# hmorimitsu/ptlflow

Measured on AMD Instinct MI355X. Metric: frame-pairs/sec, RAFT 32-iter 436x1024, higher is better.
Workload: dtype f32; 1 GPU; raft random-init (seeded), 436x1024 frame pairs, 32 iterations, fp32, batch 8/GPU, eval forward incl. encoders, mask head + convex upsample on every iteration as the reference; global_batch=8, parallelism=dp1 (independent replicas, no collectives)

## Files before the change

### include/pfk.h

```cpp
#ifndef PFK_H
#define PFK_H

#include <stdint.h>

#ifdef __cplusplus
extern "C" {
#endif

typedef void* pfk_stream_t;

enum pfk_status {
  PFK_OK = 0,
  PFK_ERR_BAD_ARG = -1,
  PFK_ERR_ALIGNMENT = -2,
  PFK_ERR_UNSUPPORTED = -3,
  PFK_ERR_LAUNCH = -4,
  PFK_ERR_DISABLED = -5
};

#define PFK_MAX_LEVELS 8
#define PFK_ABI_VERSION 7

int pfk_abi_version(void);
const char* pfk_status_string(int status);
// ... 106 lines not shown
  long long workspace_bytes;
  int cout_active;
  int cout_split;
} pfk_conv_desc;

long long pfk_conv_workspace_bytes(void);
long long pfk_conv_workspace_fault_offset(void);
int pfk_conv_ktot(const pfk_conv_desc* d);
int pfk_conv2d_f32(const pfk_conv_desc* d, pfk_stream_t stream);

#define PFK_CONV_GROUP_MAX 4
int pfk_conv2d_group_f32(const pfk_conv_desc* descs, int n, pfk_stream_t stream);

long long pfk_conv_wino_weight_floats(int cin, int cout);
int pfk_conv2d_wino_f32(const pfk_conv_desc* d, pfk_stream_t stream);

int pfk_conv2d_wino_res_f32(const pfk_conv_desc* d, pfk_stream_t stream);

int pfk_conv2d_wino_norm_f32(const pfk_conv_desc* d, const float* in_mean, const float* in_rstd, int in_relu, pfk_stream_t stream);

long long pfk_conv_wino_stats_workspace_bytes(int B, int H, int W, int cout);
int pfk_conv2d_wino_stats_f32(const pfk_conv_desc* d, const float* in_mean, const float* in_rstd, int in_relu, float eps,
                              float* out_mean, float* out_rstd, void* workspace, long long workspace_bytes, pfk_stream_t stream);

long long pfk_conv_wino1d_weight_floats(int ktot, int cout);
int pfk_conv1d_wino_f32(const pfk_conv_desc* d, pfk_stream_t stream);

int pfk_conv_ktot_bf16(const pfk_conv_desc* d);
int pfk_conv2d_bf16s(const pfk_conv_desc* d, const void* weight_planes, int nsplit, pfk_stream_t stream);

typedef struct {
  const void* ptr;
  int ld;
  int channels;
} pfk_conv_src_b16;

typedef struct {
  pfk_conv_src_b16 src[3];
  int num_src;
  int B, H, W;
  int kh, kw;
  const void* weight;
  const float* bias;
  int cout;
  int epilogue;
  int relu;
// ... 190 lines not shown
```

### ptlflow_amd/csrc/pfk_torch.cpp

```cpp
#include <torch/library.h>

#include <type_traits>
#include <vector>

#include "pfk_torch_views.h"

namespace {

void corr_volume_impl(const char* op, Elem e, const Tensor& f1, const Tensor& f2, double scale, const Tensor& out) {
  OpScope scope(f1);
  const Ptr a = dense(op, f1, "f1", e), b = dense(op, f2, "f2", e), o = dense(op, out, "out", e);
  TORCH_CHECK(f1.dim() == 3 && f2.dim() == 3 && out.dim() == 3, op, ": [B,N,D] inputs, [B,N1,N2] out");
  const int B = f1.size(0), N1 = f1.size(1), D = f1.size(2), N2 = f2.size(1);
  TORCH_CHECK(f2.size(0) == B && f2.size(2) == D && out.size(0) == B && out.size(1) == N1 && out.size(2) == N2, op, ": shape mismatch");
  if (e == B16) check_ok(pfk_corr_volume_bf16(a.raw(), D, b.raw(), D, o.raw(), B, N1, N2, D, (float)scale, cur_stream()), op);
  else check_ok(pfk_corr_volume_f32(a.f32(), D, b.f32(), D, o.f32(), B, N1, N2, D, (float)scale, cur_stream()), op);
}
void corr_volume(const Tensor& f1, const Tensor& f2, double scale, Tensor out) { corr_volume_impl("corr_volume", F32, f1, f2, scale, out); }
void corr_volume_bf16(const Tensor& f1, const Tensor& f2, double scale, Tensor out) { corr_volume_impl("corr_volume_bf16", B16, f1, f2, scale, out); }

void corr_pool2x2(const Tensor& in, Tensor out) {
  OpScope scope(in);
  const Ptr i = dense("corr_pool2x2", in, "inp", Any);
  TORCH_CHECK(in.dim() == 3, "corr_pool2x2: inp must be [M,H,W] contiguous");
// ... 286 lines not shown
  }
  check_ok(pfk_conv2d_b16(&d, cur_stream()), "conv2d_b16");
}

void conv2d_b16(at::TensorList srcs, int64_t B, int64_t H, int64_t W, int64_t kh, int64_t kw, const Tensor& weight,
                const c10::optional<Tensor>& bias, int64_t cout, int64_t epilogue, bool relu, double scale,
                const c10::optional<Tensor>& out, const c10::optional<Tensor>& h, const c10::optional<Tensor>& h_b16,
                const c10::optional<Tensor>& aux_z, const c10::optional<Tensor>& aux_rh, const c10::optional<Tensor>& residual,
                int64_t stride, bool relu_after_residual) {
  conv2d_b16_run(srcs, B, H, W, kh, kw, weight, bias, cout, epilogue, relu, scale, out, h, h_b16, aux_z, aux_rh, residual, stride,
                 relu_after_residual, false);
}

void conv2d_gelu_b16(at::TensorList srcs, int64_t B, int64_t H, int64_t W, int64_t kh, int64_t kw, const Tensor& weight,
                     const c10::optional<Tensor>& bias, int64_t cout, double scale, const Tensor& out,
                     const c10::optional<Tensor>& residual) {
  TORCH_CHECK(weight.dim() == 2, "conv2d_gelu_b16: bf16 packed weight [cout, ktot] (no batched form)");
  conv2d_b16_run(srcs, B, H, W, kh, kw, weight, bias, cout, PFK_EPI_LINEAR_GELU, false, scale, out, c10::nullopt, c10::nullopt,
                 c10::nullopt, c10::nullopt, residual, 1, false, true);
}

void debug_set_b16(int64_t cfg) { check_ok(pfk_debug_set_b16((int)cfg), "debug_set_b16"); }
void debug_set_stem_valu(int64_t on) { check_ok(pfk_debug_set_stem_valu((int)on), "debug_set_stem_valu"); }
void debug_set_cin2_valu(int64_t on) { check_ok(pfk_debug_set_cin2_valu((int)on), "debug_set_cin2_valu"); }

void conv_cin2(const Tensor& in, const Tensor& weight, const c10::optional<Tensor>& bias, Tensor out,
               int64_t B, int64_t H, int64_t W, int64_t k, bool relu) {
  OpScope scope(in);
  const Rows i = rows("conv_cin2", in, "inp", F32).expect(B * H * W, AtLeast{2});
  const Rows o = rows("conv_cin2", out, "out", Any).expect(B * H * W, AtLeast{0});
  const int cout = o.cols;
  const float* wp = dense("conv_cin2", weight, "weight [k*k,2,cout]", F32, k * k * 2 * cout).f32();
  const float* bp = dense("conv_cin2", bias, "bias", F32, AtLeast{cout}).f32();
  if (o.b16) check_ok(pfk_conv_cin2_b16(i.f32(), i.ld, wp, bp, o.raw(), o.ld, 0, B, H, W, k, cout, relu, cur_stream()), "conv_cin2 (bf16 out)");
  else check_ok(pfk_conv_cin2_f32(i.f32(), i.ld, wp, bp, o.f32(), o.ld, 0, B, H, W, k, cout, relu, cur_stream()), "conv_cin2");
}

void flow_delta(const Tensor& in, const Tensor& weight, const c10::optional<Tensor>& bias, const Tensor& coords0,
                Tensor coords1, const c10::optional<Tensor>& delta_out, const c10::optional<Tensor>& flow_out,
                const c10::optional<Tensor>& flow_out_b16) {
  OpScope scope(in);
  const float* c0 = dense("flow_delta", coords0, "coords0", F32).f32();
  TORCH_CHECK(coords0.dim() == 4 && coords0.size(1) == 2, "flow_delta: coords0 must be [B,2,h,w] contiguous");
  const int B = coords0.size(0), H = coords0.size(2), W = coords0.size(3);
  const int64_t M = (int64_t)B * H * W;
  float* c1 = dense("flow_delta", coords1, "coords1", F32, 2 * M).f32();
// ... 710 lines not shown
  m.def("corr_lookup_blocked(Tensor[] levels, int[] lvl_h, int[] lvl_w, Tensor coords, int radius, Tensor(a!) out) -> ()");
  m.def("blocked_map_elems(int H, int W) -> int", &blocked_map_elems);
  m.def("conv2d(Tensor[] srcs, int B, int H, int W, int kh, int kw, Tensor weight, Tensor? bias, int cout, "
        "int epilogue, bool relu, float scale, Tensor(a!)? out, Tensor(b!)? h, Tensor(c!)? aux_z, Tensor(d!)? aux_rh, "
        "Tensor(e!)? workspace=None, Tensor? residual=None, int stride=1, bool relu_after_residual=False, int cout_active=0, int cout_split=0) -> ()");
  m.def("conv2d_wino(Tensor src, int B, int H, int W, Tensor weight, Tensor? bias, int cout, bool relu, float scale, Tensor(a!) out, "
        "int cout_active=0) -> ()");
  m.def("conv2d_wino_norm(Tensor src, int B, int H, int W, Tensor weight, Tensor? bias, int cout, bool relu, float scale, Tensor(a!) out, "
        "Tensor in_mean, Tensor in_rstd, bool in_relu) -> ()");
  m.def("conv_wino_stats_workspace_bytes(int B, int H, int W, int cout) -> int", &conv_wino_stats_workspace_bytes);
  m.def("conv2d_wino_stats(Tensor src, int B, int H, int W, Tensor weight, Tensor? bias, int cout, Tensor(a!) out, Tensor? in_mean, "
        "Tensor? in_rstd, bool in_relu, float eps, Tensor(b!) out_mean, Tensor(c!) out_rstd, Tensor(d!) workspace) -> ()");
  m.def("conv2d_wino1d(Tensor[] srcs, int B, int H, int W, int kh, int kw, Tensor weight, Tensor? bias, int cout, int epilogue, "
        "bool relu, float scale, Tensor(a!)? out=None, Tensor(b!)? h=None, Tensor(c!)? aux_z=None, Tensor(d!)? aux_rh=None, "
        "Tensor? residual=None) -> ()");
  m.def("conv2d_wino_res(Tensor src, int B, int H, int W, Tensor weight, Tensor? bias, int cout, bool relu, float scale, Tensor(a!) out, "
        "Tensor residual, bool relu_after_residual) -> ()");
  m.def("conv2d_group(Tensor[] srcs, int B, int H, int W, int[] k, Tensor[] weights, Tensor[] biases, int[] relu, float[] scale, Tensor(a!)[] outs, Tensor[] residuals) -> ()");
  m.def("conv2d_b16(Tensor[] srcs, int B, int H, int W, int kh, int kw, Tensor weight, Tensor? bias, int cout, int epilogue, bool relu, "
        "float scale, Tensor(a!)? out, Tensor(b!)? h=None, Tensor(c!)? h_b16=None, Tensor(d!)? aux_z=None, Tensor(e!)? aux_rh=None, "
        "Tensor? residual=None, int stride=1, bool relu_after_residual=False) -> ()");
  m.def("debug_set_b16(int cfg) -> ()", &debug_set_b16);
  m.def("debug_set_stem_valu(int on) -> ()", &debug_set_stem_valu);
  m.def("debug_set_cin2_valu(int on) -> ()", &debug_set_cin2_valu);
  m.def("conv_workspace_bytes() -> int", &conv_workspace_bytes);
  m.def("conv_workspace_fault_offset() -> int", &conv_workspace_fault_offset);
  m.def("conv_cin2(Tensor inp, Tensor weight, Tensor? bias, Tensor(a!) out, int B, int H, int W, int k, bool relu) -> ()");
  m.def("flow_delta(Tensor inp, Tensor weight, Tensor? bias, Tensor coords0, Tensor(a!) coords1, Tensor(b!)? delta_out, "
        "Tensor(c!)? flow_out, Tensor(d!)? flow_out_b16=None) -> ()");
  m.def("flow_from_coords(Tensor coords0, Tensor coords1, Tensor(a!) flow_out) -> ()");
  m.def("convex_upsample(Tensor flow, Tensor mask, Tensor(a!) out) -> ()");
  m.def("convex_upsample_pm(Tensor flow_pm, Tensor mask, Tensor(a!) out) -> ()");
  m.def("convex_upsample_info_pm(Tensor flow_pm, Tensor info_pm, Tensor mask, Tensor(a!) flow_out, Tensor(b!) info_out) -> ()");
  m.def("dwconv_layernorm(Tensor inp, Tensor dw_weight, Tensor? dw_bias, Tensor ln_weight, Tensor ln_bias, float eps, Tensor(a!) out, "
        "int B, int H, int W, int k) -> ()");
  m.def("dwconv_layernorm_train(Tensor inp, Tensor dw_weight, Tensor? dw_bias, Tensor ln_weight, Tensor ln_bias, float eps, "
        "Tensor(a!) out, Tensor(b!) xhat, Tensor(c!) rstd, int B, int H, int W, int k) -> ()");
  m.def("layernorm_bwd(Tensor xhat, Tensor rstd, Tensor ln_weight, Tensor dy, Tensor(a!) du, Tensor(b!) dgamma, Tensor(c!) dbeta) -> ()");
  m.def("dwconv_bwd(Tensor inp, Tensor du, Tensor dw_weight, Tensor(a!) dx, Tensor(b!) dweight, Tensor(c!)? dbias, int B, int H, int W, "
        "int k) -> ()");
  m.def("gelu(Tensor x, Tensor(a!) y) -> ()");
  m.def("gelu_bwd(Tensor x, Tensor dy, Tensor(a!) dx) -> ()");
  m.def("dwconv_layernorm_b16(Tensor inp, Tensor dw_weight, Tensor? dw_bias, Tensor ln_weight, Tensor ln_bias, float eps, "
        "Tensor(a!) out, int B, int H, int W, int k) -> ()");
  m.def("conv2d_gelu_b16(Tensor[] srcs, int B, int H, int W, int kh, int kw, Tensor weight, Tensor? bias, int cout, float scale, "
        "Tensor(a!) out, Tensor? residual=None) -> ()");
// ... 78 lines not shown
```

### ptlflow_amd/csrc/pfk_wino.hip

```cpp
#include "pfk_gemm.h"

using namespace pfkg;

namespace {

constexpr int WT = 32;
constexpr int WN = 64;
constexpr int WK = 8;
constexpr int UIMG = 16 * WN * WK;

typedef float f32x2 __attribute__((ext_vector_type(2)));
typedef __attribute__((address_space(3))) float lfloat;
typedef __attribute__((address_space(3))) f32x2 lf32x2;
typedef __attribute__((address_space(3))) f32x4 lf32x4;

struct WinoArgs {
  const float* src; int ld;
  unsigned src_bytes;
  int H, W;
  int tw, tpi;
  int ntiles;
  int nks;
  const float* weight; unsigned w_bytes;
  const float* bias;
  int cout;
  int ncb;
  int relu; float scale;
  float* out; int out_ld, out_coff;
  unsigned out_bytes;
  const float* res; int res_ld;
  unsigned res_bytes;
  int relu2;
  int vec;
  const float* in_mean; const float* in_rstd;
  unsigned stat_bytes;
  int cin, in_relu;
  int nbi;
  double* part; long long astride;
};

constexpr unsigned T_OK = 0x80000000u, T_ROW2 = 0x40000000u, T_COL2 = 0x20000000u, T_PIX = 0x1fffffffu;
constexpr int ESZ = 64 * 32 + 4 * 16;

__device__ __forceinline__ __amdgpu_buffer_rsrc_t rsrc_n(const void* p, unsigned bytes) {
  return __builtin_amdgcn_make_buffer_rsrc(const_cast<void*>(p), 0, (int)bytes, 0x00020000);
}

__device__ __forceinline__ void wino_load_stat(__amdgpu_buffer_rsrc_t rm, __amdgpu_buffer_rsrc_t rr, unsigned soff, int ks, float (&mr)[2]) {
  mr[0] = __builtin_bit_cast(float, __builtin_amdgcn_raw_buffer_load_b32(rm, soff, ks * WK * 4, 0));
  mr[1] = __builtin_bit_cast(float, __builtin_amdgcn_raw_buffer_load_b32(rr, soff, ks * WK * 4, 0));
}

__device__ __forceinline__ void wino_load_v2(__amdgpu_buffer_rsrc_t rs, const unsigned (&voff)[16], int ks, int q, float (&d)[16]) {
  d[q] = __builtin_bit_cast(float, __builtin_amdgcn_raw_buffer_load_b32(rs, voff[q], ks * WK * 4, 0));
  d[q + 1] = __builtin_bit_cast(float, __builtin_amdgcn_raw_buffer_load_b32(rs, voff[q + 1], ks * WK * 4, 0));
}

__device__ __forceinline__ void wino_dma_u(__amdgpu_buffer_rsrc_t rw, lfloat* dst, unsigned wvoff, unsigned wk, int j) {
#if defined(__HIP_DEVICE_COMPILE__)
  __builtin_amdgcn_raw_ptr_buffer_load_lds(rw, (__attribute__((address_space(3))) void*)(dst + j * 1024), 16, wvoff, wk + j * 4096u, 0, 0);
#endif
// ... 17 lines not shown
      u0[n] = *(const lf32x2*)(aU + (x + 1) * WN * WK);
      u1[n] = *(const lf32x2*)(aU1 + (x + 1) * WN * WK);
    }
    if (more) {
      if (x < 8) wino_dma_u(rw, udst, wvoff, wk, x);
      else wino_load_v2(rs, voff, ks, 2 * (x - 8), d);
      if constexpr (NORM) {
        if (x == 8) wino_load_stat(rm, rr, soff, ks, mr);
      }
    }
    __builtin_amdgcn_sched_barrier(0);
    acc[x][0] = __builtin_amdgcn_mfma_f32_16x16x4f32(va[c][0], u0[c][0], acc[x][0], 0, 0, 0);
    acc[x][1] = __builtin_amdgcn_mfma_f32_16x16x4f32(va[c][0], u1[c][0], acc[x][1], 0, 0, 0);
    acc[x][0] = __builtin_amdgcn_mfma_f32_16x16x4f32(va[c][1], u0[c][1], acc[x][0], 0, 0, 0);
    acc[x][1] = __builtin_amdgcn_mfma_f32_16x16x4f32(va[c][1], u1[c][1], acc[x][1], 0, 0, 0);
    __builtin_amdgcn_sched_barrier(0);
  }
}

typedef __attribute__((address_space(3))) unsigned lunsigned;
typedef unsigned int u32x4v __attribute__((__vector_size__(16)));

template <bool RES, bool VEC>
__device__ __forceinline__ void wino_epi_request(const WinoArgs& a, const lunsigned* tT, int n0, unsigned (&oo)[8], f32x4 (&r4)[8]) {
  unsigned ro[8];
#pragma unroll
  for (int i = 0; i < 8; ++i) {
    oo[i] = tT[2 * i] + (unsigned)(a.out_coff + n0) * 4u;
    if constexpr (RES) ro[i] = tT[4 * WT + 2 * i] + (unsigned)n0 * 4u;
  }
  if constexpr (RES) {
    const __amdgpu_buffer_rsrc_t rr = rsrc_n(a.res, a.res_bytes);
#pragma unroll
    for (int i = 0; i < 8; ++i) {
      if constexpr (VEC) {
        r4[i] = __builtin_bit_cast(f32x4, __builtin_amdgcn_raw_buffer_load_b128(rr, ro[i], 0, 0));
      } else {
#pragma unroll
        for (int j = 0; j < 4; ++j)
          r4[i][j] = __builtin_bit_cast(float, __builtin_amdgcn_raw_buffer_load_b32(rr, n0 + j < a.cout ? ro[i] + 4u * j : OOB, 0, 0));
      }
    }
  }
}

template <bool RES, bool VEC, bool STATS>
__device__ __forceinline__ void wino_epi_store(const WinoArgs& a, const lfloat* rE, int n0, const unsigned (&oo)[8], const f32x4 (&r4)[8],
                                               double (&st)[8]) {
  const __amdgpu_buffer_rsrc_t ro = rsrc_n(a.out, a.out_bytes);
  const __amdgpu_buffer_rsrc_t rbias = rsrc_n(a.bias, a.bias != nullptr ? (unsigned)a.cout * 4u : 0u);
  float bias4[4];
#pragma unroll
  for (int j = 0; j < 4; ++j) bias4[j] = __builtin_bit_cast(float, __builtin_amdgcn_raw_buffer_load_b32(rbias, (unsigned)(n0 + j) * 4u, 0, 0));
  const float lo = a.relu ? 0.f : -__builtin_inff(), lo2 = a.relu2 ? 0.f : -__builtin_inff();
#pragma unroll
  for (int i = 0; i < 8; ++i) {
    const f32x4 y = *(const lf32x4*)(rE + i * 256 + (i >> 1) * 16);
    float v[4];
#pragma unroll
    for (int j = 0; j < 4; ++j) {
      float t = y[j] + bias4[j];
      t = (t < lo) ? lo : t;
      if constexpr (RES) {
        t = __builtin_fmaf(t, a.scale, r4[i][j]);
        t = (t < lo2) ? lo2 : t;
      } else {
        t *= a.scale;
      }
      v[j] = t;
      if constexpr (STATS) {
        const double dv = (double)((oo[i] < OOB && (VEC || n0 + j < a.cout)) ? t : 0.f);
        st[j] += dv;
        st[4 + j] = __builtin_fma(dv, dv, st[4 + j]);
      }
    }
    if constexpr (VEC) {
      __builtin_amdgcn_raw_buffer_store_b128(__builtin_bit_cast(u32x4v, (f32x4{v[0], v[1], v[2], v[3]})), ro, oo[i], 0, 0);
    } else {
#pragma unroll
      for (int j = 0; j < 4; ++j)
        __builtin_amdgcn_raw_buffer_store_b32(__builtin_bit_cast(unsigned, v[j]), ro, n0 + j < a.cout ? oo[i] + 4u * j : OOB, 0, 0);
    }
  }
}

template <bool RES, bool NORM = false, bool STATS = false>
__global__ __launch_bounds__(256, 2) void conv_gemm_wino_f32_kernel(const WinoArgs a) {
  static_assert(!(RES && STATS), "the residual form is never in front of an instance norm");
  __shared__ __attribute__((aligned(16))) float smem[2 * UIMG + 16 * WT * WK];
  lfloat* const sU = (lfloat*)smem;
  lfloat* const sV = sU + 2 * UIMG;

  const int tid = threadIdx.x, lane = tid & 63, wid = __builtin_amdgcn_readfirstlane(tid >> 6);
  const int cb = blockIdx.x % a.ncb;
  const int t0 = (blockIdx.x / a.ncb) * WT;

  const __amdgpu_buffer_rsrc_t rs = rsrc_n(a.src, a.src_bytes);
  const __amdgpu_buffer_rsrc_t rw = rsrc_n(a.weight, a.w_bytes);
  const __amdgpu_buffer_rsrc_t rm = rsrc_n(a.in_mean, NORM ? a.stat_bytes : 0u);
  const __amdgpu_buffer_rsrc_t rr = rsrc_n(a.in_rstd, NORM ? a.stat_bytes : 0u);

  const int lt = tid >> 3, cc = tid & 7;
  unsigned voff[16];
  unsigned tinfo;
  unsigned soff = 0;
  {
    int g, b, r;
    bool tok;
    if constexpr (STATS) {
      const int tb = blockIdx.x / a.ncb;
      b = tb / a.nbi;
      r = (tb - b * a.nbi) * WT + lt;
      tok = r < a.tpi;
    } else {
      g = t0 + lt;
      tok = g < a.ntiles;
      b = g / a.tpi;
      r = g - b * a.tpi;
    }
    if constexpr (NORM) soff = ((unsigned)b * (unsigned)a.cin + (unsigned)cc) * 4u;
    const int ty = r / a.tw, tx = r - ty * a.tw;
    tinfo = tok ? (T_OK | (2 * ty + 1 < a.H ? T_ROW2 : 0u) | (2 * tx + 1 < a.W ? T_COL2 : 0u) | (unsigned)((b * a.H + 2 * ty) * a.W + 2 * tx)) : 0u;
#pragma unroll
    for (int i = 0; i < 4; ++i)
#pragma unroll
      for (int j = 0; j < 4; ++j) {
        const int y = 2 * ty - 1 + i, x = 2 * tx - 1 + j;
        const bool ok = tok && (unsigned)y < (unsigned)a.H && (unsigned)x < (unsigned)a.W;
        voff[i * 4 + j] = ok ? ((unsigned)((b * a.H + y) * a.W + x) * (unsigned)a.ld + (unsigned)cc) * 4u : OOB;
      }
  }
  const int vslot = ((cc & 3) * 2 + (cc >> 2)) ^ (((lt >> 2) & 3) * 2);
  lfloat* const vdst = sV + lt * WK + vslot;
  const unsigned wvoff = (unsigned)lane * 16u;
  const unsigned wbase = (unsigned)cb * (unsigned)a.nks * (UIMG * 4u) + (unsigned)wid * 1024u;
  lfloat* const udst = sU + wid * 256;

  float d[16];
  float mr[2] = {0.f, 0.f};
  const int wt = wid & 1, wc = wid >> 1;
  const int rl = lane & 15, kq = lane >> 4;
  const lfloat* const aV = sV + (wt * 16 + rl) * WK + ((kq * 2) ^ (((rl >> 2) & 3) * 2));
  const lfloat* const aU = sU + (wc * 32 + rl) * WK + ((kq * 2) ^ (((rl >> 2) & 3) * 2));
  const lfloat* aU1 = aU + 16 * WK;
  asm volatile("" : "+v"(aU1));

  f32x4 acc[16][2];
#pragma unroll
  for (int x = 0; x < 16; ++x)
#pragma unroll
    for (int c = 0; c < 2; ++c) acc[x][c] = f32x4{0.f, 0.f, 0.f, 0.f};

#pragma unroll
  for (int j = 0; j < 8; ++j) {
    wino_dma_u(rw, udst, wvoff, wbase, j);
    wino_load_v2(rs, voff, 0, 2 * j, d);
  }
  if constexpr (NORM) wino_load_stat(rm, rr, soff, 0, mr);
  const float nlo = a.in_relu ? 0.f : -__builtin_inff();  for (int ks = 0; ks < a.nks; ++ks) {
    if constexpr (NORM) {
#pragma unroll
      for (int q = 0; q < 16; ++q) {
        const float y = __fmul_rn(__fsub_rn(d[q], mr[0]), mr[1]);
        d[q] = voff[q] == OOB ? 0.f : ((y < nlo) ? nlo : y);
      }
    }
    float t[16];
#pragma unroll
    for (int j = 0; j < 4; ++j) {
      t[0 * 4 + j] = d[0 * 4 + j] - d[2 * 4 + j];
      t[1 * 4 + j] = d[1 * 4 + j] + d[2 * 4 + j];
      t[2 * 4 + j] = d[2 * 4 + j] - d[1 * 4 + j];
      t[3 * 4 + j] = d[1 * 4 + j] - d[3 * 4 + j];
    }
#pragma unroll
    for (int i = 0; i < 4; ++i) {
      vdst[(i * 4 + 0) * WT * WK] = t[i * 4 + 0] - t[i * 4 + 2];
      vdst[(i * 4 + 1) * WT * WK] = t[i * 4 + 1] + t[i * 4 + 2];
      vdst[(i * 4 + 2) * WT * WK] = t[i * 4 + 2] - t[i * 4 + 1];
      vdst[(i * 4 + 3) * WT * WK] = t[i * 4 + 1] - t[i * 4 + 3];
    }
    asm volatile("s_waitcnt vmcnt(0) lgkmcnt(0)\n\ts_barrier" ::: "memory");
    const int ub = (ks & 1) * UIMG;
    wino_mfma<NORM>(aV, aU + ub, aU1 + ub, acc, ks + 1 < a.nks, rw, udst + (UIMG - ub), wvoff, wbase + (unsigned)(ks + 1) * (UIMG * 4u),
                    rs, voff, ks + 1, d, rm, rr, soff, mr);
    asm volatile("s_waitcnt lgkmcnt(0)\n\ts_barrier" ::: "memory");
  }

  lfloat* const sE = (lfloat*)smem + wid * ESZ;
  lunsigned* const sT = (lunsigned*)((lfloat*)smem + 4 * ESZ);
  static_assert(4 * ESZ + 8 * WT <= 2 * UIMG + 16 * WT * WK, "parking areas and offset table must fit into the loop's LDS");
  {
    const unsigned need = T_OK | ((cc & 2) ? T_ROW2 : 0u) | ((cc & 1) ? T_COL2 : 0u);
    const bool ok = (tinfo & need) == need;
    const unsigned pix = (tinfo & T_PIX) + (unsigned)(((cc >> 1) & 1) * a.W + (cc & 1));
    const unsigned po = ok ? pix * (unsigned)a.out_ld * 4u : OOB;
    const unsigned pr = ok ? pix * (unsigned)a.res_ld * 4u : OOB;
    if (cc < 4) {
      sT[cc * WT + lt] = po;
      if constexpr (RES) sT[(4 + cc) * WT + lt] = pr;
    }
  }
  asm volatile("s_waitcnt lgkmcnt(0)\n\ts_barrier" ::: "memory");

  const int prow = lane >> 3, c4 = (lane & 7) * 4;
  const int n0 = cb * WN + wc * 32 + c4;
  const lunsigned* const tT = sT + (prow & 3) * WT + wt * 16 + (lane >> 5);
  const bool vec = a.vec && cb * WN + wc * 32 + 32 <= a.cout;
  unsigned oo[8];
  f32x4 r4[8];
  if (vec) wino_epi_request<RES, true>(a, tT, n0, oo, r4);
  else wino_epi_request<RES, false>(a, tT, n0, oo, r4);

  {
    lfloat* const pE = sE + kq * (16 * 32 + 16) + rl;
#pragma unroll
    for (int c = 0; c < 2; ++c)
#pragma unroll
      for (int r = 0; r < 4; ++r) {
        float m[16];
#pragma unroll
        for (int x = 0; x < 16; ++x) m[x] = acc[x][c][r];
        float s0[4], s1[4];
#pragma unroll
        for (int j = 0; j < 4; ++j) {
          s0[j] = m[0 * 4 + j] + m[1 * 4 + j] + m[2 * 4 + j];
          s1[j] = m[1 * 4 + j] - m[2 * 4 + j] - m[3 * 4 + j];
        }
        pE[(r * 4 + 0) * 32 + c * 16] = s0[0] + s0[1] + s0[2];
        pE[(r * 4 + 1) * 32 + c * 16] = s0[1] - s0[2] - s0[3];
        pE[(r * 4 + 2) * 32 + c * 16] = s1[0] + s1[1] + s1[2];
        pE[(r * 4 + 3) * 32 + c * 16] = s1[1] - s1[2] - s1[3];
      }
  }
  const lfloat* const rE = sE + prow * 32 + c4;
  double st[8] = {0., 0., 0., 0., 0., 0., 0., 0.};
  if (vec) wino_epi_store<RES, true, STATS>(a, rE, n0, oo, r4, st);
  else wino_epi_store<RES, false, STATS>(a, rE, n0, oo, r4, st);

  if constexpr (STATS) {
    typedef __attribute__((address_space(3))) double ldouble;
    ldouble* const sS = (ldouble*)(sE) + lane * 8;
#pragma unroll
    for (int j = 0; j < 8; ++j) sS[j] = st[j];
    asm volatile("s_waitcnt lgkmcnt(0)\n\ts_barrier" ::: "memory");
    if (tid < 2 * WN) {
      const int which = tid >> 6, col = tid & 63;
      const int idx = ((col & 31) >> 2) * 8 + which * 4 + (col & 3);
      double tot[2];
#pragma unroll
      for (int w = 0; w < 2; ++w) {
        const ldouble* const p = (const ldouble*)((lfloat*)smem + ((col >> 5) * 2 + w) * ESZ) + idx;
        double s = 0.;
#pragma unroll
        for (int k = 0; k < 8; ++k) s += p[k * 64];
        tot[w] = s;
      }
      const int n = cb * WN + col;
      if (n < a.cout) a.part[which * a.astride + (long long)(blockIdx.x / a.ncb) * a.cout + n] = tot[0] + tot[1];
    }
  }
}

constexpr int WN1 = 128;
constexpr int VIMG1 = 8 * WT * WK;

struct Wino1dArgs {
  const float* src0; const float* src1;
  int ld0, ld1;
  unsigned bytes0, bytes1;
  int nks0, nks;
  int H, W;
  int L, nt;
  int ntiles;
  const float* weight; unsigned w_bytes;
  const float* bias;
  int cout, ncb;
  int relu; float scale;
  float* out; int out_ld, out_coff;
  const float* res; int res_ld;
  float* h; int h_ld;
  float* aux_z; float* aux_rh;
  int ch;
  unsigned res_bytes, h_bytes, z_bytes;
// ... 421 lines not shown
  if (d->epilogue != PFK_EPI_LINEAR) {
    a.res_bytes = d->residual ? (unsigned)(((M - 1) * d->residual_ld + d->cout) * 4) : 0u;
    a.h_bytes = (unsigned)(((M - 1) * d->h_ld + ch) * 4);
    a.z_bytes = (unsigned)(M * ch * 4);
  }
  if (vert) wino1d_launch_epi<true>(a, d->epilogue, (unsigned)nblk, static_cast<hipStream_t>(stream));
  else wino1d_launch_epi<false>(a, d->epilogue, (unsigned)nblk, static_cast<hipStream_t>(stream));
  return pfk_launch_status();
}

long long pfk_conv_wino_weight_floats(int cin, int cout) {
  if (cin <= 0 || cout <= 0 || (cin & 31)) return PFK_ERR_BAD_ARG;
  return 16LL * cin * ((cout + WN - 1) / WN * WN);
}

static inline long long wino_blocks_per_image(int H, int W) { return ((long long)((H + 1) / 2) * ((W + 1) / 2) + WT - 1) / WT; }

struct WinoFuse {
  bool norm, stats;
  const float* in_mean; const float* in_rstd; int in_relu;
  float eps; float* out_mean; float* out_rstd; void* workspace; long long workspace_bytes;
};

static int wino_launch(const pfk_conv_desc* d, bool res, pfk_stream_t stream, const WinoFuse* f = nullptr) {
  if (!d) return PFK_ERR_BAD_ARG;
  const bool norm = f && f->norm, stats = f && f->stats;
  if (norm && (!f->in_mean || !f->in_rstd)) return PFK_ERR_BAD_ARG;
  if (stats && (!f->out_mean || !f->out_rstd || !f->workspace || d->residual || d->relu_after_residual)) return PFK_ERR_BAD_ARG;
  if (d->num_src != 1 || d->kh != 3 || d->kw != 3 || d->stride > 1 || d->epilogue != PFK_EPI_LINEAR)
    return PFK_ERR_UNSUPPORTED;
  if (!res && (d->residual || d->relu_after_residual)) return PFK_ERR_UNSUPPORTED;
  if (res && (!d->residual || d->residual_ld < d->cout || (reinterpret_cast<uintptr_t>(d->residual) & 3u))) return PFK_ERR_BAD_ARG;
  const pfk_conv_src& s = d->src[0];
  if (!s.ptr || !d->weight || !d->out || d->B <= 0 || d->H <= 0 || d->W <= 0 || d->cout <= 0 || s.channels <= 0 ||
      s.ld < s.channels || d->out_coff < 0 || d->out_ld < d->out_coff + d->cout)
    return PFK_ERR_BAD_ARG;
  if (s.channels & 31) return PFK_ERR_UNSUPPORTED;
  if (!pfk_aligned16(d->weight) || (reinterpret_cast<uintptr_t>(s.ptr) & 3u) || (reinterpret_cast<uintptr_t>(d->out) & 3u))
    return PFK_ERR_ALIGNMENT;
  const long long M = (long long)d->B * d->H * d->W;
  const long long src_bytes = ((M - 1) * s.ld + s.channels) * 4;
  const long long wfloats = pfk_conv_wino_weight_floats(s.channels, d->cout);
  if (M * s.ld * 4 >= 0x7fffffffLL || wfloats * 4 >= 0x7fffffffLL) return PFK_ERR_UNSUPPORTED;
  const long long out_bytes = ((M - 1) * d->out_ld + d->out_coff + d->cout) * 4;
  const long long res_bytes = res ? ((M - 1) * d->residual_ld + d->cout) * 4 : 0;
  if (out_bytes >= 0x7fffffffLL || res_bytes >= 0x7fffffffLL) return PFK_ERR_UNSUPPORTED;
// ... 10 lines not shown
  }
  WinoArgs a{};
  a.src = s.ptr; a.ld = s.ld; a.src_bytes = (unsigned)src_bytes;
  a.H = d->H; a.W = d->W;
  a.tw = (d->W + 1) / 2;
  a.tpi = a.tw * ((d->H + 1) / 2);
  const long long ntiles = (long long)d->B * a.tpi;
  const long long nbi = wino_blocks_per_image(d->H, d->W);
  const long long nblk = (stats ? d->B * nbi : (ntiles + WT - 1) / WT) * ncb;
  if (nblk >= 0x7fffffffLL || ntiles >= 0x7fffffffLL) return PFK_ERR_UNSUPPORTED;
  a.ntiles = (int)ntiles;
  a.nks = s.channels / WK;
  a.weight = d->weight; a.w_bytes = (unsigned)(wfloats * 4);
  a.bias = d->bias;
  a.cout = d->cout;
  a.ncb = ncb;
  a.relu = d->relu ? 1 : 0; a.scale = d->scale;
  a.out = d->out; a.out_ld = d->out_ld; a.out_coff = d->out_coff; a.out_bytes = (unsigned)out_bytes;
  a.vec = pfk_aligned16(d->out + d->out_coff) && !(d->out_ld & 3) && (!res || (pfk_aligned16(d->residual) && !(d->residual_ld & 3)));
  if (norm) {
    a.in_mean = f->in_mean; a.in_rstd = f->in_rstd; a.in_relu = f->in_relu ? 1 : 0;
    a.cin = s.channels; a.stat_bytes = (unsigned)((long long)d->B * s.channels * 4);
  }
  hipStream_t st = static_cast<hipStream_t>(stream);
  if (stats) {
    a.nbi = (int)nbi;
    a.part = static_cast<double*>(f->workspace);
    a.astride = (long long)d->B * nbi * d->cout;
    if (norm) hipLaunchKernelGGL((conv_gemm_wino_f32_kernel<false, true, true>), dim3((unsigned)nblk), dim3(256), 0, st, a);
    else hipLaunchKernelGGL((conv_gemm_wino_f32_kernel<false, false, true>), dim3((unsigned)nblk), dim3(256), 0, st, a);
    return pfk_instnorm_finish_parts(a.part, d->B, a.nbi, d->cout, d->H * d->W, f->eps, f->out_mean, f->out_rstd, st);
  }
  if (norm) {
    if (res) return PFK_ERR_UNSUPPORTED;
    hipLaunchKernelGGL((conv_gemm_wino_f32_kernel<false, true, false>), dim3((unsigned)nblk), dim3(256), 0, st, a);
    return pfk_launch_status();
  }
  if (res) {
    if (d->cout_active > 0 && d->cout_active < d->cout) return PFK_ERR_UNSUPPORTED;
    a.res = d->residual; a.res_ld = d->residual_ld; a.res_bytes = (unsigned)res_bytes; a.relu2 = d->relu_after_residual ? 1 : 0;
    hipLaunchKernelGGL(conv_gemm_wino_f32_kernel<true>, dim3((unsigned)nblk), dim3(256), 0, static_cast<hipStream_t>(stream), a);
  } else {
    hipLaunchKernelGGL(conv_gemm_wino_f32_kernel<false>, dim3((unsigned)nblk), dim3(256), 0, static_cast<hipStream_t>(stream), a);
  }
  return pfk_launch_status();
}

int pfk_conv2d_wino_f32(const pfk_conv_desc* d, pfk_stream_t stream) { return wino_launch(d, false, stream); }

int pfk_conv2d_wino_res_f32(const pfk_conv_desc* d, pfk_stream_t stream) { return wino_launch(d, true, stream); }

int pfk_conv2d_wino_norm_f32(const pfk_conv_desc* d, const float* in_mean, const float* in_rstd, int in_relu, pfk_stream_t stream) {
  const WinoFuse f{true, false, in_mean, in_rstd, in_relu, 0.f, nullptr, nullptr, nullptr, 0};
  return wino_launch(d, false, stream, &f);
}

long long pfk_conv_wino_stats_workspace_bytes(int B, int H, int W, int cout) {
  if (B <= 0 || H <= 0 || W <= 0 || cout <= 0) return PFK_ERR_BAD_ARG;
  return 2LL * B * wino_blocks_per_image(H, W) * cout * (long long)sizeof(double);
}

int pfk_conv2d_wino_stats_f32(const pfk_conv_desc* d, const float* in_mean, const float* in_rstd, int in_relu, float eps,
                              float* out_mean, float* out_rstd, void* workspace, long long workspace_bytes, pfk_stream_t stream) {
  if ((in_mean == nullptr) != (in_rstd == nullptr)) return PFK_ERR_BAD_ARG;
  const WinoFuse f{in_mean != nullptr, true, in_mean, in_rstd, in_relu, eps, out_mean, out_rstd, workspace, workspace_bytes};
  return wino_launch(d, false, stream, &f);
}


}
```

Measured before the change: 126.3 frame-pairs/s.

## Make Winograd conv kernel persistent, overlapping next tile's loads with epilogue

```diff
diff --git a/include/pfk.h b/include/pfk.h
--- a/include/pfk.h
+++ b/include/pfk.h
@@ -152,6 +152,8 @@
 long long pfk_conv_wino_stats_workspace_bytes(int B, int H, int W, int cout);
 int pfk_conv2d_wino_stats_f32(const pfk_conv_desc* d, const float* in_mean, const float* in_rstd, int in_relu, float eps,
                               float* out_mean, float* out_rstd, void* workspace, long long workspace_bytes, pfk_stream_t stream);
+
+int pfk_debug_set_wino_slots(int n);
 
 long long pfk_conv_wino1d_weight_floats(int ktot, int cout);
 int pfk_conv1d_wino_f32(const pfk_conv_desc* d, pfk_stream_t stream);
diff --git a/ptlflow_amd/csrc/pfk_torch.cpp b/ptlflow_amd/csrc/pfk_torch.cpp
--- a/ptlflow_amd/csrc/pfk_torch.cpp
+++ b/ptlflow_amd/csrc/pfk_torch.cpp
@@ -332,6 +332,7 @@
 
 void debug_set_b16(int64_t cfg) { check_ok(pfk_debug_set_b16((int)cfg), "debug_set_b16"); }
 void debug_set_stem_valu(int64_t on) { check_ok(pfk_debug_set_stem_valu((int)on), "debug_set_stem_valu"); }
+void debug_set_wino_slots(int64_t n) { check_ok(pfk_debug_set_wino_slots((int)n), "debug_set_wino_slots"); }
 void debug_set_cin2_valu(int64_t on) { check_ok(pfk_debug_set_cin2_valu((int)on), "debug_set_cin2_valu"); }
 
 void conv_cin2(const Tensor& in, const Tensor& weight, const c10::optional<Tensor>& bias, Tensor out,
@@ -1088,6 +1089,7 @@
         "Tensor? residual=None, int stride=1, bool relu_after_residual=False) -> ()");
   m.def("debug_set_b16(int cfg) -> ()", &debug_set_b16);
   m.def("debug_set_stem_valu(int on) -> ()", &debug_set_stem_valu);
+  m.def("debug_set_wino_slots(int n) -> ()", &debug_set_wino_slots);
   m.def("debug_set_cin2_valu(int on) -> ()", &debug_set_cin2_valu);
   m.def("conv_workspace_bytes() -> int", &conv_workspace_bytes);
   m.def("conv_workspace_fault_offset() -> int", &conv_workspace_fault_offset);
diff --git a/ptlflow_amd/csrc/pfk_wino.hip b/ptlflow_amd/csrc/pfk_wino.hip
--- a/ptlflow_amd/csrc/pfk_wino.hip
+++ b/ptlflow_amd/csrc/pfk_wino.hip
@@ -37,6 +37,9 @@
   int cin, in_relu;
   int nbi;
   double* part; long long astride;
+  int nitems;
+  unsigned ncb_mul, tpi_mul, tw_mul, nbi_mul;
+  int ncb_sh, tpi_sh, tw_sh, nbi_sh;
 };
 
 constexpr unsigned T_OK = 0x80000000u, T_ROW2 = 0x40000000u, T_COL2 = 0x20000000u, T_PIX = 0x1fffffffu;
@@ -100,7 +103,8 @@
 typedef unsigned int u32x4v __attribute__((__vector_size__(16)));
 
 template <bool RES, bool VEC>
-__device__ __forceinline__ void wino_epi_request(const WinoArgs& a, const lunsigned* tT, int n0, unsigned (&oo)[8], f32x4 (&r4)[8]) {
+__device__ __forceinline__ void wino_epi_request(const WinoArgs& a, __amdgpu_buffer_rsrc_t rr, const lunsigned* tT, int n0,
+                                                 unsigned (&oo)[8], f32x4 (&r4)[8]) {
   unsigned ro[8];
 #pragma unroll
   for (int i = 0; i < 8; ++i) {
@@ -108,7 +112,6 @@
     if constexpr (RES) ro[i] = tT[4 * WT + 2 * i] + (unsigned)n0 * 4u;
   }
   if constexpr (RES) {
-    const __amdgpu_buffer_rsrc_t rr = rsrc_n(a.res, a.res_bytes);
 #pragma unroll
     for (int i = 0; i < 8; ++i) {
       if constexpr (VEC) {
@@ -122,18 +125,26 @@
   }
 }
 
+template <int OFF>
+__device__ __forceinline__ void wino_park(lfloat* p, float v) {
+  asm volatile("ds_write_b32 %0, %1 offset:%2" : : "v"(p), "v"(v), "n"(OFF * 4) : "memory");
+}
+template <int I>
+__device__ __forceinline__ void wino_unpark(const lfloat* rE, f32x4& y) {
+  asm volatile("ds_read_b128 %0, %1 offset:%2" : "=&v"(y) : "v"(rE), "n"((I * 256 + (I >> 1) * 16) * 4) : "memory");
+}
+
 template <bool RES, bool VEC, bool STATS>
-__device__ __forceinline__ void wino_epi_store(const WinoArgs& a, const lfloat* rE, int n0, const unsigned (&oo)[8], const f32x4 (&r4)[8],
-                                               double (&st)[8]) {
-  const __amdgpu_buffer_rsrc_t ro = rsrc_n(a.out, a.out_bytes);
-  const __amdgpu_buffer_rsrc_t rbias = rsrc_n(a.bias, a.bias != nullptr ? (unsigned)a.cout * 4u : 0u);
-  float bias4[4];
-#pragma unroll
-  for (int j = 0; j < 4; ++j) bias4[j] = __builtin_bit_cast(float, __builtin_amdgcn_raw_buffer_load_b32(rbias, (unsigned)(n0 + j) * 4u, 0, 0));
+__device__ __forceinline__ void wino_epi_store(const WinoArgs& a, __amdgpu_buffer_rsrc_t ro, const lfloat* rE, int n0,
+                                               const float (&bias4)[4], const unsigned (&oo)[8], const f32x4 (&r4)[8], double (&st)[8]) {
   const float lo = a.relu ? 0.f : -__builtin_inff(), lo2 = a.relu2 ? 0.f : -__builtin_inff();
+  f32x4 yy[8];
+  wino_unpark<0>(rE, yy[0]); wino_unpark<1>(rE, yy[1]); wino_unpark<2>(rE, yy[2]); wino_unpark<3>(rE, yy[3]);
+  wino_unpark<4>(rE, yy[4]); wino_unpark<5>(rE, yy[5]); wino_unpark<6>(rE, yy[6]); wino_unpark<7>(rE, yy[7]);
+  asm volatile("s_waitcnt lgkmcnt(0)" : "+v"(yy[0]), "+v"(yy[1]), "+v"(yy[2]), "+v"(yy[3]), "+v"(yy[4]), "+v"(yy[5]), "+v"(yy[6]), "+v"(yy[7]) : : "memory");
 #pragma unroll
   for (int i = 0; i < 8; ++i) {
-    const f32x4 y = *(const lf32x4*)(rE + i * 256 + (i >> 1) * 16);
+    const f32x4 y = yy[i];
     float v[4];
 #pragma unroll
     for (int j = 0; j < 4; ++j) {
@@ -162,80 +173,167 @@
   }
 }
 
+template <int C, int I = 0>
+__device__ __forceinline__ void wino_park_all(lfloat* pE, const float (&y)[16]) {
+  wino_park<I * 32 + C * 16>(pE, y[I]);
+  if constexpr (I + 1 < 16) wino_park_all<C, I + 1>(pE, y);
+}
+
+template <bool RES, bool STATS>
+__device__ __forceinline__ void wino_epi_finish(const WinoArgs& a, const f32x4 (&acc)[16][2], lfloat* pE, const lfloat* rE, lfloat* sE, lfloat* sV,
+                                                __amdgpu_buffer_rsrc_t ro, int n0, bool vec, const float (&bias4)[4], const unsigned (&oo)[8],
+                                                const f32x4 (&r4)[8], int tb, int cb, int tid, int lane) {
+#pragma unroll
+  for (int c = 0; c < 2; ++c) {
+    float y[16];
+#pragma unroll
+    for (int r = 0; r < 4; ++r) {
+      float m[16];
+#pragma unroll
+      for (int x = 0; x < 16; ++x) m[x] = acc[x][c][r];
+      float s0[4], s1[4];
+#pragma unroll
+      for (int j = 0; j < 4; ++j) {
+        s0[j] = m[0 * 4 + j] + m[1 * 4 + j] + m[2 * 4 + j];
+        s1[j] = m[1 * 4 + j] - m[2 * 4 + j] - m[3 * 4 + j];
+      }
+      y[r * 4 + 0] = s0[0] + s0[1] + s0[2];
+      y[r * 4 + 1] = s0[1] - s0[2] - s0[3];
+      y[r * 4 + 2] = s1[0] + s1[1] + s1[2];
+      y[r * 4 + 3] = s1[1] - s1[2] - s1[3];
+    }
+    if (c == 0) wino_park_all<0>(pE, y);
+    else wino_park_all<1>(pE, y);
+  }
+  double st[8] = {0., 0., 0., 0., 0., 0., 0., 0.};
+  if (vec) wino_epi_store<RES, true, STATS>(a, ro, rE, n0, bias4, oo, r4, st);
+  else wino_epi_store<RES, false, STATS>(a, ro, rE, n0, bias4, oo, r4, st);
+
+  if constexpr (STATS) {
+    typedef __attribute__((address_space(3))) double ldouble;
+    ldouble* const sS = (ldouble*)(sE) + lane * 8;
+#pragma unroll
+    for (int j = 0; j < 8; ++j) sS[j] = st[j];
+    asm volatile("s_waitcnt lgkmcnt(0)\n\ts_barrier" ::: "memory");
+    if (tid < 2 * WN) {
+      const int which = tid >> 6, col = tid & 63;
+      const int idx = ((col & 31) >> 2) * 8 + which * 4 + (col & 3);
+      double tot[2];
+#pragma unroll
+      for (int w = 0; w < 2; ++w) {
+        const ldouble* const p = (const ldouble*)(sV + ((col >> 5) * 2 + w) * ESZ) + idx;
+        double s = 0.;
+#pragma unroll
+        for (int k = 0; k < 8; ++k) s += p[k * 64];
+        tot[w] = s;
+      }
+      const int n = cb * WN + col;
+      if (n < a.cout) a.part[which * a.astride + (long long)tb * a.cout + n] = tot[0] + tot[1];
+    }
+  }
+}
+
+template <bool NORM, bool STATS>
+__device__ __forceinline__ void wino_item(const WinoArgs& a, int tb, int lt, int cc, unsigned (&voff)[16], unsigned& tinfo, unsigned& soff) {
+  int b, r;
+  bool tok;
+  if constexpr (STATS) {
+    b = (int)fastdiv_u32((unsigned)tb, a.nbi_mul, a.nbi_sh);
+    r = (tb - b * a.nbi) * WT + lt;
+    tok = r < a.tpi;
+  } else {
+    const int g = tb * WT + lt;
+    tok = g < a.ntiles;
+    b = (int)fastdiv_u32((unsigned)g, a.tpi_mul, a.tpi_sh);
+    r = g - b * a.tpi;
+  }
+  if constexpr (NORM) soff = ((unsigned)b * (unsigned)a.cin + (unsigned)cc) * 4u;
+  const int ty = (int)fastdiv_u32((unsigned)r, a.tw_mul, a.tw_sh), tx = r - ty * a.tw;
+  tinfo = tok ? (T_OK | (2 * ty + 1 < a.H ? T_ROW2 : 0u) | (2 * tx + 1 < a.W ? T_COL2 : 0u) | (unsigned)((b * a.H + 2 * ty) * a.W + 2 * tx)) : 0u;
+#pragma unroll
+  for (int i = 0; i < 4; ++i)
+#pragma unroll
+    for (int j = 0; j < 4; ++j) {
+      const int y = 2 * ty - 1 + i, x = 2 * tx - 1 + j;
+      const bool ok = tok && (unsigned)y < (unsigned)a.H && (unsigned)x < (unsigned)a.W;
+      voff[i * 4 + j] = ok ? ((unsigned)((b * a.H + y) * a.W + x) * (unsigned)a.ld + (unsigned)cc) * 4u : OOB;
+    }
+}
+
+template <bool NORM>
+__device__ __forceinline__ void wino_first(__amdgpu_buffer_rsrc_t rw, lfloat* udst, unsigned wvoff, unsigned wbase, __amdgpu_buffer_rsrc_t rs,
+                                           const unsigned (&voff)[16], float (&d)[16], __amdgpu_buffer_rsrc_t rm, __amdgpu_buffer_rsrc_t rr,
+                                           unsigned soff, float (&mr)[2]) {
+#pragma unroll
+  for (int j = 0; j < 8; ++j) {
+    wino_dma_u(rw, udst, wvoff, wbase, j);
+    wino_load_v2(rs, voff, 0, 2 * j, d);
+  }
+  if constexpr (NORM) wino_load_stat(rm, rr, soff, 0, mr);
+}
+
 template <bool RES, bool NORM = false, bool STATS = false>
 __global__ __launch_bounds__(256, 2) void conv_gemm_wino_f32_kernel(const WinoArgs a) {
   static_assert(!(RES && STATS), "the residual form is never in front of an instance norm");
-  __shared__ __attribute__((aligned(16))) float smem[2 * UIMG + 16 * WT * WK];
+  constexpr int VSZ = 16 * WT * WK, UB1 = UIMG + VSZ;
+  __shared__ __attribute__((aligned(16))) float smem[2 * UIMG + VSZ];
   lfloat* const sU = (lfloat*)smem;
-  lfloat* const sV = sU + 2 * UIMG;
+  lfloat* const sV = sU + UIMG;
 
   const int tid = threadIdx.x, lane = tid & 63, wid = __builtin_amdgcn_readfirstlane(tid >> 6);
-  const int cb = blockIdx.x % a.ncb;
-  const int t0 = (blockIdx.x / a.ncb) * WT;
 
   const __amdgpu_buffer_rsrc_t rs = rsrc_n(a.src, a.src_bytes);
   const __amdgpu_buffer_rsrc_t rw = rsrc_n(a.weight, a.w_bytes);
   const __amdgpu_buffer_rsrc_t rm = rsrc_n(a.in_mean, NORM ? a.stat_bytes : 0u);
   const __amdgpu_buffer_rsrc_t rr = rsrc_n(a.in_rstd, NORM ? a.stat_bytes : 0u);
-
+  const __amdgpu_buffer_rsrc_t ro = rsrc_n(a.out, a.out_bytes);
+  const __amdgpu_buffer_rsrc_t rres = rsrc_n(a.res, RES ? a.res_bytes : 0u);
+  const __amdgpu_buffer_rsrc_t rbias = rsrc_n(a.bias, a.bias != nullptr ? (unsigned)a.cout * 4u : 0u);
   const int lt = tid >> 3, cc = tid & 7;
-  unsigned voff[16];
-  unsigned tinfo;
-  unsigned soff = 0;
-  {
-    int g, b, r;
-    bool tok;
-    if constexpr (STATS) {
-      const int tb = blockIdx.x / a.ncb;
-      b = tb / a.nbi;
-      r = (tb - b * a.nbi) * WT + lt;
-      tok = r < a.tpi;
-    } else {
-      g = t0 + lt;
-      tok = g < a.ntiles;
-      b = g / a.tpi;
-      r = g - b * a.tpi;
-    }
-    if constexpr (NORM) soff = ((unsigned)b * (unsigned)a.cin + (unsigned)cc) * 4u;
-    const int ty = r / a.tw, tx = r - ty * a.tw;
-    tinfo = tok ? (T_OK | (2 * ty + 1 < a.H ? T_ROW2 : 0u) | (2 * tx + 1 < a.W ? T_COL2 : 0u) | (unsigned)((b * a.H + 2 * ty) * a.W + 2 * tx)) : 0u;
-#pragma unroll
-    for (int i = 0; i < 4; ++i)
-#pragma unroll
-      for (int j = 0; j < 4; ++j) {
-        const int y = 2 * ty - 1 + i, x = 2 * tx - 1 + j;
-        const bool ok = tok && (unsigned)y < (unsigned)a.H && (unsigned)x < (unsigned)a.W;
-        voff[i * 4 + j] = ok ? ((unsigned)((b * a.H + y) * a.W + x) * (unsigned)a.ld + (unsigned)cc) * 4u : OOB;
-      }
-  }
   const int vslot = ((cc & 3) * 2 + (cc >> 2)) ^ (((lt >> 2) & 3) * 2);
   lfloat* const vdst = sV + lt * WK + vslot;
   const unsigned wvoff = (unsigned)lane * 16u;
-  const unsigned wbase = (unsigned)cb * (unsigned)a.nks * (UIMG * 4u) + (unsigned)wid * 1024u;
   lfloat* const udst = sU + wid * 256;
-
-  float d[16];
-  float mr[2] = {0.f, 0.f};
   const int wt = wid & 1, wc = wid >> 1;
   const int rl = lane & 15, kq = lane >> 4;
   const lfloat* const aV = sV + (wt * 16 + rl) * WK + ((kq * 2) ^ (((rl >> 2) & 3) * 2));
   const lfloat* const aU = sU + (wc * 32 + rl) * WK + ((kq * 2) ^ (((rl >> 2) & 3) * 2));
   const lfloat* aU1 = aU + 16 * WK;
   asm volatile("" : "+v"(aU1));
+  lfloat* const sE = sV + wid * ESZ;
+  lunsigned* const sT = (lunsigned*)(sV + 4 * ESZ);
+  static_assert(4 * ESZ + 8 * WT <= VSZ + UIMG, "parking areas and offset table must fit into V and one U buffer");
+  const int prow = lane >> 3, c4 = (lane & 7) * 4;
+  const lunsigned* const tT = sT + (prow & 3) * WT + wt * 16 + (lane >> 5);
+  lfloat* const pE = sE + kq * (16 * 32 + 16) + rl;
+  const lfloat* const rE = sE + prow * 32 + c4;
+  const float nlo = a.in_relu ? 0.f : -__builtin_inff();
+
+  int item = blockIdx.x;
+  int tb = (int)fastdiv_u32((unsigned)item, a.ncb_mul, a.ncb_sh);
+  int cb = item - tb * a.ncb;
+  unsigned voff[16];
+  unsigned tinfo;
+  unsigned soff = 0;
+  wino_item<NORM, STATS>(a, tb, lt, cc, voff, tinfo, soff);
+  unsigned wbase = (unsigned)cb * (unsigned)a.nks * (UIMG * 4u) + (unsigned)wid * 1024u;
+  float d[16];
+  float mr[2] = {0.f, 0.f};
+  wino_first<NORM>(rw, udst, wvoff, wbase, rs, voff, d, rm, rr, soff, mr);
 
   f32x4 acc[16][2];
+  int n0;
+  bool vec;
+  float bias4[4];
+  unsigned oo[8];
+  f32x4 r4[8];
+  for (;;) {
 #pragma unroll
   for (int x = 0; x < 16; ++x)
 #pragma unroll
     for (int c = 0; c < 2; ++c) acc[x][c] = f32x4{0.f, 0.f, 0.f, 0.f};
 
-#pragma unroll
-  for (int j = 0; j < 8; ++j) {
-    wino_dma_u(rw, udst, wvoff, wbase, j);
-    wino_load_v2(rs, voff, 0, 2 * j, d);
-  }
-  if constexpr (NORM) wino_load_stat(rm, rr, soff, 0, mr);
-  const float nlo = a.in_relu ? 0.f : -__builtin_inff();  for (int ks = 0; ks < a.nks; ++ks) {
+  for (int ks = 0; ks < a.nks; ++ks) {
     if constexpr (NORM) {
 #pragma unroll
       for (int q = 0; q < 16; ++q) {
@@ -259,15 +357,12 @@
       vdst[(i * 4 + 3) * WT * WK] = t[i * 4 + 1] - t[i * 4 + 3];
     }
     asm volatile("s_waitcnt vmcnt(0) lgkmcnt(0)\n\ts_barrier" ::: "memory");
-    const int ub = (ks & 1) * UIMG;
-    wino_mfma<NORM>(aV, aU + ub, aU1 + ub, acc, ks + 1 < a.nks, rw, udst + (UIMG - ub), wvoff, wbase + (unsigned)(ks + 1) * (UIMG * 4u),
+    const int ub = (ks & 1) * UB1;
+    wino_mfma<NORM>(aV, aU + ub, aU1 + ub, acc, ks + 1 < a.nks, rw, udst + (UB1 - ub), wvoff, wbase + (unsigned)(ks + 1) * (UIMG * 4u),
                     rs, voff, ks + 1, d, rm, rr, soff, mr);
     asm volatile("s_waitcnt lgkmcnt(0)\n\ts_barrier" ::: "memory");
   }
 
-  lfloat* const sE = (lfloat*)smem + wid * ESZ;
-  lunsigned* const sT = (lunsigned*)((lfloat*)smem + 4 * ESZ);
-  static_assert(4 * ESZ + 8 * WT <= 2 * UIMG + 16 * WT * WK, "parking areas and offset table must fit into the loop's LDS");
   {
     const unsigned need = T_OK | ((cc & 2) ? T_ROW2 : 0u) | ((cc & 1) ? T_COL2 : 0u);
     const bool ok = (tinfo & need) == need;
@@ -281,63 +376,29 @@
   }
   asm volatile("s_waitcnt lgkmcnt(0)\n\ts_barrier" ::: "memory");
 
-  const int prow = lane >> 3, c4 = (lane & 7) * 4;
-  const int n0 = cb * WN + wc * 32 + c4;
-  const lunsigned* const tT = sT + (prow & 3) * WT + wt * 16 + (lane >> 5);
-  const bool vec = a.vec && cb * WN + wc * 32 + 32 <= a.cout;
-  unsigned oo[8];
-  f32x4 r4[8];
-  if (vec) wino_epi_request<RES, true>(a, tT, n0, oo, r4);
-  else wino_epi_request<RES, false>(a, tT, n0, oo, r4);
-
-  {
-    lfloat* const pE = sE + kq * (16 * 32 + 16) + rl;
-#pragma unroll
-    for (int c = 0; c < 2; ++c)
-#pragma unroll
-      for (int r = 0; r < 4; ++r) {
-        float m[16];
-#pragma unroll
-        for (int x = 0; x < 16; ++x) m[x] = acc[x][c][r];
-        float s0[4], s1[4];
-#pragma unroll
-        for (int j = 0; j < 4; ++j) {
-          s0[j] = m[0 * 4 + j] + m[1 * 4 + j] + m[2 * 4 + j];
-          s1[j] = m[1 * 4 + j] - m[2 * 4 + j] - m[3 * 4 + j];
-        }
-        pE[(r * 4 + 0) * 32 + c * 16] = s0[0] + s0[1] + s0[2];
-        pE[(r * 4 + 1) * 32 + c * 16] = s0[1] - s0[2] - s0[3];
-        pE[(r * 4 + 2) * 32 + c * 16] = s1[0] + s1[1] + s1[2];
-        pE[(r * 4 + 3) * 32 + c * 16] = s1[1] - s1[2] - s1[3];
-      }
-  }
-  const lfloat* const rE = sE + prow * 32 + c4;
-  double st[8] = {0., 0., 0., 0., 0., 0., 0., 0.};
-  if (vec) wino_epi_store<RES, true, STATS>(a, rE, n0, oo, r4, st);
-  else wino_epi_store<RES, false, STATS>(a, rE, n0, oo, r4, st);
-
-  if constexpr (STATS) {
-    typedef __attribute__((address_space(3))) double ldouble;
-    ldouble* const sS = (ldouble*)(sE) + lane * 8;
-#pragma unroll
-    for (int j = 0; j < 8; ++j) sS[j] = st[j];
-    asm volatile("s_waitcnt lgkmcnt(0)\n\ts_barrier" ::: "memory");
-    if (tid < 2 * WN) {
-      const int which = tid >> 6, col = tid & 63;
-      const int idx = ((col & 31) >> 2) * 8 + which * 4 + (col & 3);
-      double tot[2];
-#pragma unroll
-      for (int w = 0; w < 2; ++w) {
-        const ldouble* const p = (const ldouble*)((lfloat*)smem + ((col >> 5) * 2 + w) * ESZ) + idx;
-        double s = 0.;
-#pragma unroll
-        for (int k = 0; k < 8; ++k) s += p[k * 64];
-        tot[w] = s;
-      }
-      const int n = cb * WN + col;
-      if (n < a.cout) a.part[which * a.astride + (long long)(blockIdx.x / a.ncb) * a.cout + n] = tot[0] + tot[1];
-    }
-  }
+  n0 = cb * WN + wc * 32 + c4;
+  vec = a.vec && cb * WN + wc * 32 + 32 <= a.cout;
+#pragma unroll
+  for (int j = 0; j < 4; ++j) bias4[j] = __builtin_bit_cast(float, __builtin_amdgcn_raw_buffer_load_b32(rbias, (unsigned)(n0 + j) * 4u, 0, 0));
+  if (vec) wino_epi_request<RES, true>(a, rres, tT, n0, oo, r4);
+  else wino_epi_request<RES, false>(a, rres, tT, n0, oo, r4);
+
+  if ((unsigned)item + gridDim.x >= (unsigned)a.nitems) break;
+  __builtin_amdgcn_sched_barrier(0);
+
+  const int tb_c = tb, cb_c = cb;
+  item += (int)gridDim.x;
+  tb = (int)fastdiv_u32((unsigned)item, a.ncb_mul, a.ncb_sh);
+  cb = item - tb * a.ncb;
+  wino_item<NORM, STATS>(a, tb, lt, cc, voff, tinfo, soff);
+  wbase = (unsigned)cb * (unsigned)a.nks * (UIMG * 4u) + (unsigned)wid * 1024u;
+  wino_first<NORM>(rw, udst, wvoff, wbase, rs, voff, d, rm, rr, soff, mr);
+  __builtin_amdgcn_sched_barrier(0);
+
+  wino_epi_finish<RES, STATS>(a, acc, pE, rE, sE, sV, ro, n0, vec, bias4, oo, r4, tb_c, cb_c, tid, lane);
+  asm volatile("s_waitcnt lgkmcnt(0)\n\ts_barrier" ::: "memory");
+  }
+  wino_epi_finish<RES, STATS>(a, acc, pE, rE, sE, sV, ro, n0, vec, bias4, oo, r4, tb, cb, tid, lane);
 }
 
 constexpr int WN1 = 128;
@@ -805,6 +866,8 @@
   float eps; float* out_mean; float* out_rstd; void* workspace; long long workspace_bytes;
 };
 
+static int g_wino_slots = 0;
+
 static int wino_launch(const pfk_conv_desc* d, bool res, pfk_stream_t stream, const WinoFuse* f = nullptr) {
   if (!d) return PFK_ERR_BAD_ARG;
   const bool norm = f && f->norm, stats = f && f->stats;
@@ -861,26 +924,33 @@
     a.in_mean = f->in_mean; a.in_rstd = f->in_rstd; a.in_relu = f->in_relu ? 1 : 0;
     a.cin = s.channels; a.stat_bytes = (unsigned)((long long)d->B * s.channels * 4);
   }
+  a.nitems = (int)nblk;
+  const long long slots = g_wino_slots > 0 ? g_wino_slots : nblk;
+  const unsigned grid = (unsigned)(nblk < slots ? nblk : slots);
+  fastdiv_make((unsigned)ncb, a.ncb_mul, a.ncb_sh);
+  fastdiv_make((unsigned)a.tpi, a.tpi_mul, a.tpi_sh);
+  fastdiv_make((unsigned)a.tw, a.tw_mul, a.tw_sh);
+  fastdiv_make((unsigned)nbi, a.nbi_mul, a.nbi_sh);
   hipStream_t st = static_cast<hipStream_t>(stream);
   if (stats) {
     a.nbi = (int)nbi;
     a.part = static_cast<double*>(f->workspace);
     a.astride = (long long)d->B * nbi * d->cout;
-    if (norm) hipLaunchKernelGGL((conv_gemm_wino_f32_kernel<false, true, true>), dim3((unsigned)nblk), dim3(256), 0, st, a);
-    else hipLaunchKernelGGL((conv_gemm_wino_f32_kernel<false, false, true>), dim3((unsigned)nblk), dim3(256), 0, st, a);
+    if (norm) hipLaunchKernelGGL((conv_gemm_wino_f32_kernel<false, true, true>), dim3(grid), dim3(256), 0, st, a);
+    else hipLaunchKernelGGL((conv_gemm_wino_f32_kernel<false, false, true>), dim3(grid), dim3(256), 0, st, a);
     return pfk_instnorm_finish_parts(a.part, d->B, a.nbi, d->cout, d->H * d->W, f->eps, f->out_mean, f->out_rstd, st);
   }
   if (norm) {
     if (res) return PFK_ERR_UNSUPPORTED;
-    hipLaunchKernelGGL((conv_gemm_wino_f32_kernel<false, true, false>), dim3((unsigned)nblk), dim3(256), 0, st, a);
+    hipLaunchKernelGGL((conv_gemm_wino_f32_kernel<false, true, false>), dim3(grid), dim3(256), 0, st, a);
     return pfk_launch_status();
   }
   if (res) {
     if (d->cout_active > 0 && d->cout_active < d->cout) return PFK_ERR_UNSUPPORTED;
     a.res = d->residual; a.res_ld = d->residual_ld; a.res_bytes = (unsigned)res_bytes; a.relu2 = d->relu_after_residual ? 1 : 0;
-    hipLaunchKernelGGL(conv_gemm_wino_f32_kernel<true>, dim3((unsigned)nblk), dim3(256), 0, static_cast<hipStream_t>(stream), a);
+    hipLaunchKernelGGL(conv_gemm_wino_f32_kernel<true>, dim3(grid), dim3(256), 0, st, a);
   } else {
-    hipLaunchKernelGGL(conv_gemm_wino_f32_kernel<false>, dim3((unsigned)nblk), dim3(256), 0, static_cast<hipStream_t>(stream), a);
+    hipLaunchKernelGGL(conv_gemm_wino_f32_kernel<false>, dim3(grid), dim3(256), 0, st, a);
   }
   return pfk_launch_status();
 }
@@ -906,5 +976,10 @@
   return wino_launch(d, false, stream, &f);
 }
 
-
-}
+int pfk_debug_set_wino_slots(int n) {
+  if (!pfk_debug_knobs_enabled()) return PFK_ERR_DISABLED;
+  g_wino_slots = n < -1 ? 0 : n;
+  return PFK_OK;
+}
+
+}
```

Result: no change. 125.8 frame-pairs/s (-0.5%).
